# nutdb/nutdb

Hardware: AMD Instinct MI355X
Metric: rows/sec filter->group-by on 1e9-row i64/f64; achieved HBM GB/s vs peak (higher is better)
Workload: dtype i64+f64

## Files before the change

### nutdb_amd/csrc/msd_sort.hip

```cpp
#include <algorithm>
#include <cstdlib>
#include <utility>
#include <vector>

#include "common.hpp"
#include "sort.hpp"

namespace nut {

constexpr int MH_THREADS = 256;
constexpr uint32_t MH_TILE = 1u << 16;
constexpr uint32_t MH_HTILE = 1u << 18;
constexpr int MH_LOADS = 16;
constexpr int MS_THREADS = 1024;
constexpr int MS_ITEMS = 14;
constexpr uint32_t MS_TILE = MS_THREADS * MS_ITEMS;
constexpr int MS_BITS = 9;
constexpr int MS_BINS = 1 << MS_BITS;
static_assert(MS_BINS <= MS_THREADS, "one scan thread per digit");
constexpr int LS_NCLS = 4;
constexpr int LS_S_THREADS = 256, LS_S_ITEMS = 8;
constexpr int LS_M_THREADS = 512, LS_M_ITEMS = 10;
constexpr int LS_M2_THREADS = 512, LS_M2_ITEMS = 12;
constexpr int LS_L_THREADS = 1024, LS_L_ITEMS = 24;
constexpr uint64_t LS_S_CAP = LS_S_THREADS * LS_S_ITEMS;
constexpr uint64_t LS_M_CAP = LS_M_THREADS * LS_M_ITEMS;
constexpr uint64_t LS_M2_CAP = LS_M2_THREADS * LS_M2_ITEMS;
constexpr uint64_t LS_CAP = LS_L_THREADS * LS_L_ITEMS;
__host__ __device__ constexpr int ls_class(uint64_t c) {
  return c <= LS_S_CAP ? 0 : c <= LS_M_CAP ? 1 : c <= LS_M2_CAP ? 2 : c <= LS_CAP ? 3 : LS_NCLS;
}

constexpr uint64_t kSameDst = ~0ull;
struct MsSeg {
  uint64_t start, count;
  uint32_t buf;
  uint32_t aux;
  uint64_t dst = kSameDst;
  uint64_t base = 0;
};
struct MsBufs {
  const uint64_t *in;
  uint64_t *a;
  uint64_t *b;
  uint64_t *c;
};
__device__ __forceinline__ uint64_t ms_dst_off(const MsSeg &g) { return g.dst == kSameDst ? g.start : g.dst; }
struct MsDigit {
  uint64_t base;
  int shift;
  uint32_t mask;
  __device__ __forceinline__ uint32_t operator()(uint64_t k) const { return (uint32_t)((k - base) >> shift) & mask; }
  static constexpr bool kCheck = false;
  static constexpr int kAux = 0;
  __device__ __forceinline__ void setup(uint8_t *) const {}
  __device__ __forceinline__ uint32_t operator()(uint64_t k, const uint8_t *) const { return (*this)(k); }
  uint64_t maxx = ~0ull;
};
struct MsSplit {
  int ns, sbits;
  int64_t e[63];
  const uint8_t *tab;
  static constexpr bool kCheck = false;
  static constexpr int kAux = 4096;
  __device__ __forceinline__ void setup(uint8_t *s) const {
    for (int i = threadIdx.x; i < kAux; i += blockDim.x) s[i] = tab[i];
  }
  __device__ __forceinline__ uint32_t operator()(uint64_t k, const uint8_t *lds) const {
    const uint32_t t = lds[(k ^ 0x8000000000000000ull) >> 52];
    uint32_t d = t & 63u;
    if (t & 0x80u)
      while (d < (uint32_t)ns && (int64_t)k >= e[d]) ++d;
    const uint32_t h = (uint32_t)(k ^ (k >> 29) ^ (k >> 43));
    return (d << sbits) | (h & ((1u << sbits) - 1u));
  }
};
struct MsMap {
  uint64_t base;
  uint32_t mul, lim;
  int t, dshift;
  uint64_t maxx;
  static constexpr bool kCheck = true;
  static constexpr int kAux = 0;
  __device__ __forceinline__ void setup(uint8_t *) const {}
  __device__ __forceinline__ uint32_t operator()(uint64_t k) const {
    return (__umulhi((uint32_t)((k - base) >> t), mul) >> dshift) & (MS_BINS - 1);
  }
  __device__ __forceinline__ uint32_t operator()(uint64_t k, const uint8_t *) const { return (*this)(k); }
};

__device__ __forceinline__ const uint64_t *ms_src(const MsBufs &bf, uint32_t buf) {
  return buf == 0 ? bf.in : (buf == 1 ? bf.a : (buf == 2 ? bf.b : bf.c));
}

template <class DG>
__global__ __launch_bounds__(MH_THREADS) void ms_hist_kernel(MsBufs bf, const MsSeg *__restrict__ segs,
                                                             const uint32_t *__restrict__ tile_seg, DG dg0,
                                                             uint64_t flip, unsigned long long *__restrict__ hist,
                                                             unsigned long long *__restrict__ minmax) {
  __shared__ uint32_t h[MS_BINS];
  __shared__ uint8_t s_aux[DG::kAux > 0 ? DG::kAux : 4];
  const int tid = threadIdx.x;
  dg0.setup(s_aux);
  auto dg = [&](uint64_t k) { return dg0(k, s_aux); };
  for (int i = tid; i < MS_BINS; i += MH_THREADS) h[i] = 0;
  __syncthreads();
  const uint32_t s = tile_seg[blockIdx.x];
  const MsSeg sg = segs[s];
  const uint64_t lo = (uint64_t)(blockIdx.x - sg.aux) * MH_HTILE;
  const uint32_t cnt = (uint32_t)min<uint64_t>(MH_HTILE, sg.count - lo);
  const uint64_t *src = ms_src(bf, sg.buf) + sg.start + lo;
  const uint64_t f = sg.buf == 0 ? flip : 0;
  uint64_t vmin = ~0ull, vmax = 0;
  for (uint32_t i = tid; i < cnt; i += MH_THREADS * MH_LOADS) {
    uint64_t k[MH_LOADS];
#pragma unroll
// ... 5 lines not shown
        atomicAdd(&h[dg(k[j])], 1u);
        vmin = k[j] < vmin ? k[j] : vmin;
        vmax = k[j] > vmax ? k[j] : vmax;
      }
    }
  }
  if (minmax) {
#pragma unroll
    for (int off = 32; off >= 1; off >>= 1) {
      const uint64_t a = __shfl_xor(vmin, off, 64), b = __shfl_xor(vmax, off, 64);
      vmin = a < vmin ? a : vmin;
      vmax = b > vmax ? b : vmax;
    }
    if ((tid & 63) == 0) {
      atomicMin(&minmax[0], (unsigned long long)vmin);
      atomicMax(&minmax[1], (unsigned long long)vmax);
    }
  }
  __syncthreads();
  for (int i = tid; i < MS_BINS; i += MH_THREADS)
    if (h[i]) atomicAdd(&hist[(uint64_t)s * MS_BINS + i], (unsigned long long)h[i]);
}

__device__ __forceinline__ uint64_t *ms_dst(const MsBufs &bf, uint32_t buf, int dst_buf) {
  return dst_buf == 1 ? bf.a : dst_buf == 2 ? bf.b : dst_buf == 3 ? bf.c : (buf == 2 ? bf.a : bf.b);
}
constexpr uint64_t kSkipRun = ~0ull;

template <int H, class DG, int T = MS_THREADS>
__global__ __launch_bounds__(T, 2048 / T) void ms_scatter_kernel(MsBufs bf, const MsSeg *__restrict__ segs,
                                                                   const uint32_t *__restrict__ tile_seg, uint32_t ntiles,
                                                                   DG dg0, uint64_t flip,
                                                                   unsigned long long *__restrict__ cursor,
                                                                   int dst_buf = -1, uint64_t ocap = 0,
                                                                   unsigned long long *__restrict__ oflag = nullptr) {
  constexpr int ITEMS = MS_ITEMS * H;
  constexpr uint32_t STAGE = (uint32_t)T * MS_ITEMS;
  constexpr uint32_t TILE = STAGE * H;
  static_assert(MS_BINS <= T, "one scan thread per digit");
  static_assert(TILE <= 65536, "16-bit ranks");
  __shared__ uint64_t s_keys[STAGE];
  __shared__ uint32_t s_cnt[MS_BINS];
  __shared__ uint32_t s_tex[MS_BINS];
  __shared__ uint64_t s_gb[MS_BINS];
  __shared__ uint32_t s_wsum[MS_BINS / kWave];
  __shared__ uint8_t s_aux[DG::kAux > 0 ? DG::kAux : 4];
  const int tid = threadIdx.x, lane = tid & 63, wave = tid >> 6;
  dg0.setup(s_aux);
  auto dg = [&](uint64_t k) { return dg0(k, s_aux); };
  uint32_t t = blockIdx.x;
  uint64_t key[ITEMS];
  auto load = [&](uint32_t tt, const MsSeg g) {
    const uint64_t lo = (uint64_t)(tt - g.aux) * TILE;
    const uint32_t cn = (uint32_t)min<uint64_t>(TILE, g.count - lo);
    const uint64_t *sp = ms_src(bf, g.buf) + g.start + lo;
    int tq = tid;
    asm volatile("" : "+v"(tq));
#pragma unroll
    for (int i = 0; i < ITEMS; ++i) key[i] = __builtin_nontemporal_load(sp + min((uint32_t)(i * T + tq), cn - 1));
  };
  uint32_t s = tile_seg[t];
  MsSeg sg = segs[s];
  load(t, sg);
  for (;;) {
    int tid_ = tid;
    asm volatile("" : "+v"(tid_));
    const int tid = tid_;
    if (sg.buf == 0 && flip) {
#pragma unroll
      for (int i = 0; i < ITEMS; ++i) key[i] ^= flip;
    }
    const uint64_t lo = (uint64_t)(t - sg.aux) * TILE;
    const uint32_t cnt = (uint32_t)min<uint64_t>(TILE, sg.count - lo);
    uint64_t *dst = ms_dst(bf, sg.buf, dst_buf);
    const uint32_t next = t + gridDim.x;
    const uint32_t ns = next < ntiles ? tile_seg[next] : 0;
    if (tid < MS_BINS) s_cnt[tid] = 0;
    __syncthreads();
    uint32_t rk[ITEMS / 2];
#pragma unroll
    for (int i = 0; i < ITEMS; i += 2) rk[i / 2] = 0;
    bool bad = false;
#pragma unroll
    for (int i = 0; i < ITEMS; ++i) {
      const uint32_t idx = (uint32_t)i * T + tid;
      if (idx < cnt) {
        rk[i / 2] |= atomicAdd(&s_cnt[dg(key[i])], 1u) << (16 * (i & 1));
        if constexpr (DG::kCheck) bad |= key[i] - dg0.base > dg0.maxx;
      }
      if (i % 8 == 7) __builtin_amdgcn_sched_barrier(0);
    }
    if constexpr (DG::kCheck)
      if (__ballot(bad) && lane == 0) atomicOr(oflag, 1ull);
    __syncthreads();
    uint32_t c = 0, incl = 0;
    if (tid < MS_BINS) {
      c = s_cnt[tid];
      incl = c;
#pragma unroll
      for (int off = 1; off < 64; off <<= 1) {
        const uint32_t y = __shfl_up(incl, off, 64);
        if (lane >= off) incl += y;
      }
      if (lane == 63) s_wsum[wave] = incl;
    }
    __syncthreads();
    if (tid < MS_BINS) {
      uint32_t add = 0;
#pragma unroll
      for (int w = 0; w < MS_BINS / kWave; ++w) add += (w < wave) ? s_wsum[w] : 0u;
      const uint32_t tex = incl - c + add;
      s_tex[tid] = tex;
      const uint64_t gb = c ? (uint64_t)atomicAdd(&cursor[(uint64_t)s * MS_BINS + tid], (unsigned long long)c) : 0;
      const bool over = ocap && c && gb + c > ((uint64_t)s * MS_BINS + tid + 1) * ocap;
      if (over) atomicOr(oflag, 1ull);
      s_gb[tid] = over ? kSkipRun : gb - tex;
    }
    __syncthreads();
#pragma unroll
    for (int i = 0; i < ITEMS; i += 2) {
      const uint32_t s0 = s_tex[dg(key[i])] + (rk[i / 2] & 0xFFFFu);
      const uint32_t s1 = s_tex[dg(key[i + 1])] + (rk[i / 2] >> 16);
      rk[i / 2] = (s0 & 0xFFFFu) | (s1 << 16);
      if (i % 8 == 6) __builtin_amdgcn_sched_barrier(0);
    }
    MsSeg nsg = sg;
#pragma unroll
    for (int h = 0; h < H; ++h) {
      if (h) __syncthreads();
#pragma unroll
      for (int i = 0; i < ITEMS; ++i) {
        const uint32_t idx = (uint32_t)i * T + tid;
        const uint32_t slot = (rk[i / 2] >> (16 * (i & 1))) & 0xFFFFu;
        if (idx < cnt && (H == 1 || slot / STAGE == (uint32_t)h)) s_keys[slot % STAGE] = key[i];
      }
      if (h == H - 1 && next < ntiles) {
        __builtin_amdgcn_sched_barrier(0);
        nsg = segs[ns];
        load(next, nsg);
      }
      __syncthreads();
#pragma unroll(H == 1 ? MS_ITEMS : 2)
      for (int i = 0; i < MS_ITEMS; ++i) {
        const uint32_t j = (uint32_t)i * T + tid, jj = j + (uint32_t)h * STAGE;
        if (jj < cnt) {
          const uint64_t k = s_keys[j];
          const uint64_t g = s_gb[dg(k)];
          if (g != kSkipRun) dst[g + jj] = k;
        }
      }
    }
    if (next >= ntiles) break;
    __syncthreads();
    t = next;
    s = ns;
    sg = nsg;
  }
}

__global__ __launch_bounds__(MS_BINS) void ms_plan_kernel(const MsSeg *__restrict__ segs,
                                                          const unsigned long long *__restrict__ hist, int hi,
                                                          uint64_t base,
                                                          unsigned long long *__restrict__ cursor,
                                                          MsSeg *__restrict__ lists, uint64_t cap,
                                                          unsigned int *__restrict__ counts) {
  __shared__ unsigned long long s_wsum[MS_BINS / kWave];
  const int d = threadIdx.x, lane = d & 63, wave = d >> 6;
  const MsSeg sg = segs[blockIdx.x];
  const uint64_t c = hist[(uint64_t)blockIdx.x * MS_BINS + d];
  uint64_t incl = c;
#pragma unroll
  for (int off = 1; off < 64; off <<= 1) {
    const uint64_t y = __shfl_up(incl, off, 64);
    if (lane >= off) incl += y;
  }
  if (lane == 63) s_wsum[wave] = incl;
  __syncthreads();
  uint64_t add = 0;
#pragma unroll
  for (int w = 0; w < MS_BINS / kWave; ++w) add += (w < wave) ? s_wsum[w] : 0ull;
  const uint64_t start = sg.start + incl - c + add;
// ... 777 lines not shown
    launch_class<LS_M_THREADS, LS_M_ITEMS, false>(c, bf, d, n, flip, fb);
  else if (cls == 2)
    launch_class<LS_M2_THREADS, LS_M2_ITEMS, false>(c, bf, d, n, flip, fb);
  else
    launch_class<LS_L_THREADS, LS_L_ITEMS, false>(c, bf, d, n, flip, fb);
  NUT_HIP(hipGetLastError());
  return NUT_OK;
}

static nut_status launch_local(nut_ctx *c, MetaArena &ar, const MsBufs &bf, uint64_t flip,
                               const std::vector<MsSeg> &segs, int cls) {
  if (segs.empty()) return NUT_OK;
  MsSeg *d;
  nut_status s = ar.upload(segs, &d);
  if (s) return s;
  uint32_t *fb = (uint32_t *)ar.alloc((segs.size() + 1) * 4);
  NUT_HIP(hipMemsetAsync(fb, 0, 4, c->stream));
  return launch_local_dev(c, bf, flip, d, (unsigned)segs.size(), fb, cls);
}


static constexpr int ms_halves() { return 2; }

static void launch_scatter(hipStream_t st, unsigned grid, const MsBufs &bf, const MsSeg *segs, const uint32_t *tiles,
                           uint32_t ntiles, const MsDigit &dg, uint64_t flip, unsigned long long *cur) {
  hipLaunchKernelGGL((ms_scatter_kernel<ms_halves(), MsDigit>), dim3(grid), dim3(MS_THREADS), 0, st, bf, segs, tiles, ntiles, dg,
                     flip, cur);
}

static nut_status device_level(nut_ctx *c, MetaArena &ar, const MsBufs &bf, const MsDigit &dg, uint64_t flip,
                               std::vector<MsSeg> &big, std::vector<MsSeg> &over) {
  hipStream_t st = c->stream;
  over.clear();
  std::vector<uint32_t> tiles;
  const uint64_t nht = tile_table(big, MH_HTILE, tiles);
  std::vector<uint32_t> stiles;
  std::vector<MsSeg> sbig = big;
  const uint64_t nst = tile_table(sbig, MS_TILE * ms_halves(), stiles);
  if (nht > 0x7FFFFFFFull || nst > 0x7FFFFFFFull) return fail(NUT_ERR_UNSUPPORTED, "nut_sort_i64: too many tiles");
  const uint64_t ns = big.size(), cap = ns * MS_BINS;
  const size_t hbytes = ns * MS_BINS * 8;
  nut_status s = ar.begin(2 * MetaArena::align(ns * sizeof(MsSeg)) + MetaArena::align(tiles.size() * 4) +
                          MetaArena::align(stiles.size() * 4) + 2 * MetaArena::align(hbytes) +
                          MetaArena::align((LS_NCLS + 1) * cap * sizeof(MsSeg)) +
                          LS_NCLS * MetaArena::align((cap + 1) * 4) + 1024);
  if (s) return s;
  MsSeg *dseg, *dsseg;
  uint32_t *dtile, *dstile;
  if ((s = ar.upload(big, &dseg)) || (s = ar.upload(tiles, &dtile)) || (s = ar.upload(sbig, &dsseg)) ||
      (s = ar.upload(stiles, &dstile)))
    return s;
  unsigned long long *dhist = (unsigned long long *)ar.alloc(hbytes);
  unsigned long long *dcur = (unsigned long long *)ar.alloc(hbytes);
  MsSeg *lists = (MsSeg *)ar.alloc((LS_NCLS + 1) * cap * sizeof(MsSeg));
  unsigned int *counts = (unsigned int *)ar.alloc(4 * (LS_NCLS + 1));
  uint32_t *fb[LS_NCLS];
  for (auto &f : fb) f = (uint32_t *)ar.alloc((cap + 1) * 4);
  NUT_HIP(hipMemsetAsync(dhist, 0, hbytes, st));
  NUT_HIP(hipMemsetAsync(counts, 0, 4 * (LS_NCLS + 1), st));
  uint64_t total = 0;
  for (const MsSeg &sg : big) total += sg.count;
  hipLaunchKernelGGL(ms_hist_kernel<MsDigit>, dim3((unsigned)nht), dim3(MH_THREADS), 0, st, bf, (const MsSeg *)dseg,
                     (const uint32_t *)dtile, dg, flip, dhist, (unsigned long long *)nullptr);
  hipLaunchKernelGGL(ms_plan_kernel, dim3((unsigned)ns), dim3(MS_BINS), 0, st, (const MsSeg *)dseg,
                     (const unsigned long long *)dhist, dg.shift, dg.base, dcur, lists, cap, counts);
  NUT_HIP(hipGetLastError());
  hipEvent_t ev = nullptr;
  NUT_HIP(hipEventCreateWithFlags(&ev, hipEventDisableTiming));
  uint32_t *hc = (uint32_t *)c->host_pinned;
  hipError_t e = hipMemcpyAsync(hc, counts, 4 * (LS_NCLS + 1), hipMemcpyDeviceToHost, st);
  if (e == hipSuccess) e = hipEventRecord(ev, st);
  if (e == hipSuccess)
    launch_scatter(st, (unsigned)std::min<uint64_t>(nst, (uint64_t)c->num_cus), bf, (const MsSeg *)dsseg,
                   (const uint32_t *)dstile, (uint32_t)nst, dg, flip, dcur);
  if (e == hipSuccess) e = hipGetLastError();
  if (e == hipSuccess) e = hipEventSynchronize(ev);
  (void)hipEventDestroy(ev);
  if (e != hipSuccess) return hip_fail(e, "nut_sort_i64 (device-planned level)");
  uint32_t cnt[LS_NCLS + 1];
  for (int k = 0; k <= LS_NCLS; ++k) cnt[k] = hc[k];
  c->sort_bytes += 8 * total + 16 * total;
  ++c->sort_levels;
  for (int cls = LS_NCLS - 1; cls >= 0; --cls)
    if ((s = launch_local_dev(c, bf, flip, lists + (uint64_t)cls * cap, cnt[cls], fb[cls], cls))) return s;
  if (cnt[LS_NCLS]) {
    over.resize(cnt[LS_NCLS]);
    NUT_HIP(hipMemcpyAsync(over.data(), lists + (uint64_t)LS_NCLS * cap, cnt[LS_NCLS] * sizeof(MsSeg),
                           hipMemcpyDeviceToHost, st));
    NUT_HIP(hipStreamSynchronize(st));
  }
  uint64_t over_keys = 0;
  for (const MsSeg &sg : over) over_keys += sg.count;
  c->sort_bytes += 16 * (total - over_keys);
  return NUT_OK;
}

constexpr uint64_t kCappedMin = 1ull << 25;

template <class DG, int T>
static void capped_scatter_t(hipStream_t st, unsigned grid, const MsBufs &bf, const MsSeg *segs, const uint32_t *tiles,
                             uint32_t nt, const DG &dg, uint64_t flip, unsigned long long *cur, int dst_buf,
                             uint64_t ocap, unsigned long long *oflag) {
  hipLaunchKernelGGL((ms_scatter_kernel<ms_halves(), DG, T>), dim3(grid), dim3(T), 0, st, bf, segs, tiles, nt, dg, flip,
                     cur, dst_buf, ocap, oflag);
}
template <class DG>
static void capped_scatter(nut_ctx *c, uint64_t nt, const MsBufs &bf, const MsSeg *segs, const uint32_t *tiles,
                           const DG &dg, uint64_t flip, unsigned long long *cur, int dst_buf, uint64_t ocap,
                           unsigned long long *oflag) {
  const bool half = c->opt[NUT_OPT_SORT_BD] == 512;
  const unsigned grid = (unsigned)std::min<uint64_t>(nt, (uint64_t)c->num_cus * (half ? 2 : 1));
  if (half)
    capped_scatter_t<DG, 512>(c->stream, grid, bf, segs, tiles, (uint32_t)nt, dg, flip, cur, dst_buf, ocap, oflag);
  else
    capped_scatter_t<DG, MS_THREADS>(c->stream, grid, bf, segs, tiles, (uint32_t)nt, dg, flip, cur, dst_buf, ocap, oflag);
}

static bool capped_map(uint64_t lo, uint64_t hi, MsMap &m) {
  if (hi < lo || hi - lo < (1ull << 18)) return false;
  const uint64_t span = hi - lo;
  const int bw = 64 - __builtin_clzll(span);
  const int t = bw > 32 ? bw - 32 : 0;
  const uint64_t lim = span >> t;
  const uint64_t mul = (1ull << 50) / (lim + 1);
  m = MsMap{lo, (uint32_t)mul, (uint32_t)lim, t, 9, ((lim + 1) << t) - 1};
  return true;
}
static uint32_t capped_cell(const MsMap &m, uint64_t k) {
  return (uint32_t)(((uint64_t)(uint32_t)((k - m.base) >> m.t) * m.mul) >> 32);
}

static nut_status msd_sort_capped(nut_ctx *c, const int64_t *in, int64_t *out, uint64_t n, uint64_t flip,
                                  const uint64_t *bounds) {
  hipStream_t st = c->stream;
  constexpr uint32_t kSample = 16384;
  MetaArena ar{c};
  nut_status s = ar.begin(MetaArena::align(kSample * 8) + 1024);
  if (s) return s;
// ... 20 lines not shown
    if (!capped_map(lo, hi, m0)) return NUT_ERR_CAPACITY;
    std::vector<uint32_t> h0(MS_BINS, 0), h1(MS_BINS, 0);
    for (uint64_t k : samp) {
      if (k < lo || k > hi) return NUT_ERR_CAPACITY;
      const uint32_t cell = capped_cell(m0, k);
      ++h0[cell >> MS_BITS];
      ++h1[cell & (MS_BINS - 1)];
    }
    const uint32_t lim = 2 * kSample / MS_BINS;
    for (int d = 0; d < MS_BINS; ++d)
      if (h0[d] > lim || h1[d] > lim) return NUT_ERR_CAPACITY;
  }
  auto reserve = [&](Scratch &sc, size_t bytes) -> nut_status {
    if (sc.reserve(bytes, false) == NUT_OK) return NUT_OK;
    (void)hipGetLastError();
    c->sort_tmp2.release();
    return NUT_ERR_CAPACITY;
  };
  const uint64_t ocap0 = ((n / MS_BINS) * 11 / 10 + 2 * MS_TILE + 31) & ~31ull;
  if ((s = reserve(c->sort_tmp, (size_t)MS_BINS * ocap0 * 8))) return s;
  const MsBufs bf0{(const uint64_t *)in, (uint64_t *)out, (uint64_t *)c->sort_tmp.ptr, nullptr};
  std::vector<MsSeg> one{MsSeg{0, n, 0, 0}};
  std::vector<uint32_t> tiles;
  const uint32_t stile = (c->opt[NUT_OPT_SORT_BD] == 512 ? 512u : (uint32_t)MS_THREADS) * MS_ITEMS * ms_halves();
  const uint64_t nt0 = tile_table(one, stile, tiles);
  if (nt0 > 0x7FFFFFFFull) return fail(NUT_ERR_UNSUPPORTED, "nut_sort_i64: too many tiles");
  std::vector<uint64_t> cur0(MS_BINS + 1, 0);
  for (int d = 0; d < MS_BINS; ++d) cur0[d] = (uint64_t)d * ocap0;
  s = ar.begin(MetaArena::align(sizeof(MsSeg)) + MetaArena::align(tiles.size() * 4) +
               MetaArena::align(cur0.size() * 8));
  if (s) return s;
  MsSeg *dseg;
  uint32_t *dtile;
  uint64_t *dcur0;
  if ((s = ar.upload(one, &dseg)) || (s = ar.upload(tiles, &dtile)) || (s = ar.upload(cur0, &dcur0))) return s;
  const bool ident = m0.base == 0 && m0.t == 32 && m0.mul == (1u << 18);
  unsigned long long *dc0 = (unsigned long long *)dcur0, *of0 = (unsigned long long *)(dcur0 + MS_BINS);
  if (ident)
    capped_scatter(c, nt0, bf0, dseg, dtile, MsDigit{0, 64 - MS_BITS, MS_BINS - 1}, flip, dc0, 2, ocap0, of0);
  else
    capped_scatter(c, nt0, bf0, dseg, dtile, m0, flip, dc0, 2, ocap0, of0);
  NUT_HIP(hipGetLastError());
  std::vector<uint64_t> end0(MS_BINS + 1);
  NUT_HIP(hipMemcpyAsync(end0.data(), dcur0, end0.size() * 8, hipMemcpyDeviceToHost, st));
  NUT_HIP(hipStreamSynchronize(st));
  if (end0[MS_BINS]) return NUT_ERR_CAPACITY;
  std::vector<MsSeg> segs(MS_BINS);
  std::vector<uint64_t> dbase(MS_BINS);
  uint64_t cmax = 0, run = 0;
  for (int d = 0; d < MS_BINS; ++d) {
    const uint64_t cnt = end0[d] - cur0[d];
    segs[d] = MsSeg{cur0[d], cnt, 2, 0};
    dbase[d] = run;
    run += cnt;
    cmax = std::max(cmax, cnt);
  }
  const uint64_t ocap1 = ((cmax / MS_BINS) * 23 / 20 + 64 + 1) & ~1ull;
  if ((s = reserve(c->sort_tmp2, (size_t)MS_BINS * MS_BINS * ocap1 * 8))) return s;
  const MsBufs bf{(const uint64_t *)in, (uint64_t *)out, (uint64_t *)c->sort_tmp.ptr, (uint64_t *)c->sort_tmp2.ptr};
  const uint64_t nt1 = tile_table(segs, stile, tiles);
  if (nt1 > 0x7FFFFFFFull) return fail(NUT_ERR_UNSUPPORTED, "nut_sort_i64: too many tiles");
  const uint64_t nr = (uint64_t)MS_BINS * MS_BINS, lcap = nr;
  std::vector<uint64_t> cur1(nr + 1, 0);
  for (uint64_t r = 0; r < nr; ++r) cur1[r] = r * ocap1;
  s = ar.begin(MetaArena::align(segs.size() * sizeof(MsSeg)) + MetaArena::align(tiles.size() * 4) +
               MetaArena::align(cur1.size() * 8) + MetaArena::align(dbase.size() * 8) +
               MetaArena::align(LS_NCLS * lcap * sizeof(MsSeg)) + LS_NCLS * MetaArena::align((lcap + 1) * 4) + 1024);
  if (s) return s;
  MsSeg *dsegs;
  uint32_t *dt1;
  uint64_t *dcur1, *ddb;
  if ((s = ar.upload(segs, &dsegs)) || (s = ar.upload(tiles, &dt1)) || (s = ar.upload(cur1, &dcur1)) ||
      (s = ar.upload(dbase, &ddb)))
    return s;
  MsSeg *lists = (MsSeg *)ar.alloc(LS_NCLS * lcap * sizeof(MsSeg));
  unsigned int *counts = (unsigned int *)ar.alloc(4 * LS_NCLS);
  uint32_t *fb[LS_NCLS];
  for (auto &f : fb) f = (uint32_t *)ar.alloc((lcap + 1) * 4);
  NUT_HIP(hipMemsetAsync(counts, 0, 4 * LS_NCLS, st));
  MsMap m1 = m0;
  m1.dshift = 0;
  m1.maxx = ~0ull;
  unsigned long long *dc1 = (unsigned long long *)dcur1, *of1 = (unsigned long long *)(dcur1 + nr);
  if (ident)
    capped_scatter(c, nt1, bf, dsegs, dt1, MsDigit{0, 64 - 2 * MS_BITS, MS_BINS - 1}, flip, dc1, 3, ocap1, of1);
  else
    capped_scatter(c, nt1, bf, dsegs, dt1, m1, flip, dc1, 3, ocap1, of1);
  hipLaunchKernelGGL(ms_plan_capped_kernel, dim3(MS_BINS), dim3(MS_BINS), 0, st, (const unsigned long long *)dcur1,
                     (const uint64_t *)ddb, ocap1, m0, lists, lcap, counts, (unsigned long long *)(dcur1 + nr));
  NUT_HIP(hipGetLastError());
  uint64_t *hc = c->host_pinned;
  static_assert(4 * LS_NCLS <= 16, "class counts in the first two pinned words");
  NUT_HIP(hipMemcpyAsync(hc, counts, 4 * LS_NCLS, hipMemcpyDeviceToHost, st));
  NUT_HIP(hipMemcpyAsync(hc + 2, dcur1 + nr, 8, hipMemcpyDeviceToHost, st));
  NUT_HIP(hipStreamSynchronize(st));
  if (hc[2]) return NUT_ERR_CAPACITY;
  const uint32_t *cnt = (const uint32_t *)hc;
  uint32_t ncls[LS_NCLS];
  for (int k = 0; k < LS_NCLS; ++k) ncls[k] = cnt[k];
  for (int cls = LS_NCLS - 1; cls >= 0; --cls)
    if ((s = launch_local_dev(c, bf, flip, lists + (uint64_t)cls * lcap, ncls[cls], fb[cls], cls))) return s;
  c->sort_bytes = 48 * n;
  c->sort_levels = 2;
  return NUT_OK;
}

nut_status msd_sort_i64(nut_ctx *c, const int64_t *in, int64_t *out, uint64_t n, uint64_t flip,
                        const uint64_t *bounds) {
  hipStream_t st = c->stream;
  c->sort_bytes = 0;
// ... 93 lines not shown
    for (size_t i = 0; i < big.size(); ++i) {
      const uint64_t *h = &hist[i * MS_BINS];
      int nz = 0;
      for (int d = 0; d < MS_BINS; ++d) nz += h[d] != 0;
      if (nz <= 1) {
        classify(big[i]);
      } else {
        scat.push_back(big[i]);
        scat_hist.insert(scat_hist.end(), h, h + MS_BINS);
      }
    }
    if (!scat.empty()) {
      cursor.resize(scat.size() * MS_BINS);
      for (size_t i = 0; i < scat.size(); ++i) {
        uint64_t run = scat[i].start;
        const uint32_t nb = scat[i].buf == 2 ? 1u : 2u;
        for (int d = 0; d < MS_BINS; ++d) {
          const uint64_t cnt = scat_hist[i * MS_BINS + d];
          cursor[i * MS_BINS + d] = run;
          if (cnt) classify(MsSeg{run, cnt, nb, 0});
          run += cnt;
        }
      }
      const uint64_t nst = tile_table(scat, MS_TILE * ms_halves(), tiles);
      if (nst > 0x7FFFFFFFull) return fail(NUT_ERR_UNSUPPORTED, "nut_sort_i64: too many tiles");
      s = ar.begin(MetaArena::align(scat.size() * sizeof(MsSeg)) + MetaArena::align(tiles.size() * 4) +
                   MetaArena::align(cursor.size() * 8));
      if (s) return s;
      MsSeg *dsc;
      uint32_t *dt;
      uint64_t *dcur;
      if ((s = ar.upload(scat, &dsc)) || (s = ar.upload(tiles, &dt)) || (s = ar.upload(cursor, &dcur))) return s;
      for (const MsSeg &sg : scat) c->sort_bytes += 16 * sg.count;
      ++c->sort_levels;
      const unsigned sgrid = (unsigned)std::min<uint64_t>(nst, (uint64_t)c->num_cus);
      launch_scatter(st, sgrid, bf, (const MsSeg *)dsc, (const uint32_t *)dt, (uint32_t)nst, dg, flip,
                     (unsigned long long *)dcur);
      NUT_HIP(hipGetLastError());
    }
    big.swap(next);
    const int w = std::min(MS_BITS, hi);
    dg = MsDigit{dg.base, hi - w, (1u << w) - 1u};
    break;
  }
  for (std::vector<MsSeg> over; !big.empty(); big.swap(over)) {
    if (dg.mask == 0) {
      done.insert(done.end(), big.begin(), big.end());
      break;
    }
    if ((s = device_level(c, ar, bf, dg, flip, big, over))) return s;
    const int hi = dg.shift, w = std::min(MS_BITS, hi);
    dg = MsDigit{dg.base, hi - w, (1u << w) - 1u};
  }
  size_t total = 256;
  for (auto &v : small) total += MetaArena::align(v.size() * sizeof(MsSeg)) + MetaArena::align((v.size() + 1) * 4);
  std::vector<uint32_t> ctiles;
  const uint64_t nct = tile_table(done, MH_TILE, ctiles);
  total += MetaArena::align(done.size() * sizeof(MsSeg)) + MetaArena::align(ctiles.size() * 4);
  s = ar.begin(total);
  if (s) return s;
// ... 93 lines not shown
```

Before: 131.9 billion.

## Add carry-granule MSD scatter that writes only aligned runs per digit

Moves the scatter kernel into a header and adds a carry mode. Each block holds back partial runs per digit in LDS and writes to global memory only in multiples of an 8-key granule, flushing the leftovers on a segment's last tile. A blocked tile assignment keeps consecutive tiles of one segment on the same block, so the carries stay valid. The goal is to cut partial-line writes and write amplification in HBM, at the cost of more LDS, a more complex scan, slightly smaller tiles (13 items per thread) and aligned overflow capacity.

```diff
diff --git a/nutdb_amd/csrc/msd_scatter.hpp b/nutdb_amd/csrc/msd_scatter.hpp
--- /dev/null
+++ b/nutdb_amd/csrc/msd_scatter.hpp
@@ -0,0 +1,288 @@
+#pragma once
+#include "common.hpp"
+
+namespace nut {
+
+constexpr int MS_THREADS = 1024;
+constexpr int MS_ITEMS = 14;
+constexpr uint32_t MS_TILE = MS_THREADS * MS_ITEMS;
+constexpr int MS_BITS = 9;
+constexpr int MS_BINS = 1 << MS_BITS;
+static_assert(MS_BINS <= MS_THREADS, "one scan thread per digit");
+
+constexpr uint64_t kSameDst = ~0ull;
+struct MsSeg {
+  uint64_t start, count;
+  uint32_t buf;
+  uint32_t aux;
+  uint64_t dst = kSameDst;
+  uint64_t base = 0;
+};
+struct MsBufs {
+  const uint64_t *in;
+  uint64_t *a;
+  uint64_t *b;
+  uint64_t *c;
+};
+__device__ __forceinline__ uint64_t ms_dst_off(const MsSeg &g) { return g.dst == kSameDst ? g.start : g.dst; }
+struct MsDigit {
+  uint64_t base;
+  int shift;
+  uint32_t mask;
+  __device__ __forceinline__ uint32_t operator()(uint64_t k) const { return (uint32_t)((k - base) >> shift) & mask; }
+  static constexpr bool kCheck = false;
+  static constexpr int kAux = 0;
+  __device__ __forceinline__ void setup(uint8_t *) const {}
+  __device__ __forceinline__ uint32_t operator()(uint64_t k, const uint8_t *) const { return (*this)(k); }
+  uint64_t maxx = ~0ull;
+};
+struct MsSplit {
+  int ns, sbits;
+  int64_t e[63];
+  const uint8_t *tab;
+  static constexpr bool kCheck = false;
+  static constexpr int kAux = 4096;
+  __device__ __forceinline__ void setup(uint8_t *s) const {
+    for (int i = threadIdx.x; i < kAux; i += blockDim.x) s[i] = tab[i];
+  }
+  __device__ __forceinline__ uint32_t operator()(uint64_t k, const uint8_t *lds) const {
+    const uint32_t t = lds[(k ^ 0x8000000000000000ull) >> 52];
+    uint32_t d = t & 63u;
+    if (t & 0x80u)
+      while (d < (uint32_t)ns && (int64_t)k >= e[d]) ++d;
+    const uint32_t h = (uint32_t)(k ^ (k >> 29) ^ (k >> 43));
+    return (d << sbits) | (h & ((1u << sbits) - 1u));
+  }
+};
+struct MsMap {
+  uint64_t base;
+  uint32_t mul, lim;
+  int t, dshift;
+  uint64_t maxx;
+  static constexpr bool kCheck = true;
+  static constexpr int kAux = 0;
+  __device__ __forceinline__ void setup(uint8_t *) const {}
+  __device__ __forceinline__ uint32_t operator()(uint64_t k) const {
+    return (__umulhi((uint32_t)((k - base) >> t), mul) >> dshift) & (MS_BINS - 1);
+  }
+  __device__ __forceinline__ uint32_t operator()(uint64_t k, const uint8_t *) const { return (*this)(k); }
+};
+
+__device__ __forceinline__ const uint64_t *ms_src(const MsBufs &bf, uint32_t buf) {
+  return buf == 0 ? bf.in : (buf == 1 ? bf.a : (buf == 2 ? bf.b : bf.c));
+}
+
+__device__ __forceinline__ uint64_t *ms_dst(const MsBufs &bf, uint32_t buf, int dst_buf) {
+  return dst_buf == 1 ? bf.a : dst_buf == 2 ? bf.b : dst_buf == 3 ? bf.c : (buf == 2 ? bf.a : bf.b);
+}
+constexpr uint64_t kSkipRun = ~0ull;
+
+template <int H, class DG, int T = MS_THREADS, int L = 0, bool BLK = (L > 0), int I1 = MS_ITEMS>
+__global__ __launch_bounds__(T, 2048 / T) void ms_scatter_kernel(MsBufs bf, const MsSeg *__restrict__ segs,
+                                                                   const uint32_t *__restrict__ tile_seg, uint32_t ntiles,
+                                                                   DG dg0, uint64_t flip,
+                                                                   unsigned long long *__restrict__ cursor,
+                                                                   int dst_buf = -1, uint64_t ocap = 0,
+                                                                   unsigned long long *__restrict__ oflag = nullptr) {
+  constexpr int ITEMS = I1 * H;
+  constexpr uint32_t TILE = (uint32_t)T * ITEMS;
+  constexpr uint32_t CARW = L ? L - 1 : 1;
+  constexpr uint32_t STAGE = L ? (TILE + MS_BINS * CARW + H - 1) / H : (uint32_t)T * I1;
+  constexpr int WI = (STAGE + T - 1) / T;
+  static_assert(MS_BINS <= T, "one scan thread per digit");
+  static_assert(L ? STAGE * H + L <= 32768 : TILE <= 65536, "16-bit slots (L > 0: 15 bits)");
+  static_assert(ITEMS % 2 == 0, "ranks in 16-bit pairs");
+  static_assert((L & (L - 1)) == 0 && L <= 128, "the carry granule is a power of two");
+  constexpr uint64_t kM48 = 0xFFFFFFFFFFFFull, kNoRun48 = 0x800000000000ull;
+  __shared__ uint64_t s_keys[STAGE];
+  __shared__ uint32_t s_cnt[MS_BINS];
+  __shared__ uint32_t s_tex[L ? 1 : MS_BINS];
+  __shared__ uint64_t s_gb[MS_BINS];
+  __shared__ uint32_t s_wsum[MS_BINS / kWave];
+  __shared__ uint8_t s_aux[DG::kAux > 0 ? DG::kAux : 4];
+  __shared__ uint64_t s_car[L ? MS_BINS * CARW : 1];
+  __shared__ uint32_t s_ccnt[L ? MS_BINS : 1];
+  __shared__ uint64_t s_sl[L ? MS_BINS : 1];
+  __shared__ uint32_t s_tot[2];
+  const int tid = threadIdx.x, lane0 = tid & 63, wave0 = tid >> 6;
+  dg0.setup(s_aux);
+  auto dg = [&](uint64_t k) { return dg0(k, s_aux); };
+  const uint32_t per = (ntiles + gridDim.x - 1) / gridDim.x;
+  uint32_t t = BLK ? blockIdx.x * per : blockIdx.x;
+  const uint32_t tend = BLK ? min(ntiles, t + per) : ntiles;
+  if (BLK && t >= tend) return;
+  if (L && tid < MS_BINS) s_ccnt[tid] = 0;
+  uint64_t key[ITEMS];
+  auto load = [&](uint32_t tt, const MsSeg g) {
+    const uint64_t lo = (uint64_t)(tt - g.aux) * TILE;
+    const uint32_t cn = (uint32_t)min<uint64_t>(TILE, g.count - lo);
+    const uint64_t *sp = ms_src(bf, g.buf) + g.start + lo;
+    int tq = tid;
+    asm volatile("" : "+v"(tq));
+#pragma unroll
+    for (int i = 0; i < ITEMS; ++i) key[i] = __builtin_nontemporal_load(sp + min((uint32_t)(i * T + tq), cn - 1));
+  };
+  uint32_t s = tile_seg[t];
+  MsSeg sg = segs[s];
+  load(t, sg);
+  for (;;) {
+    int tid_ = tid;
+    asm volatile("" : "+v"(tid_));
+    const int tid = tid_;
+    const int lane = L ? tid & 63 : lane0, wave = L ? tid >> 6 : wave0;
+    if (sg.buf == 0 && flip) {
+#pragma unroll
+      for (int i = 0; i < ITEMS; ++i) key[i] ^= flip;
+    }
+    const uint64_t lo = (uint64_t)(t - sg.aux) * TILE;
+    const uint32_t cnt = (uint32_t)min<uint64_t>(TILE, sg.count - lo);
+    uint64_t *dst = ms_dst(bf, sg.buf, dst_buf);
+    const uint32_t next = BLK ? t + 1 : t + gridDim.x;
+    const uint32_t ns = next < tend ? tile_seg[next] : 0;
+    const bool last = next >= tend || ns != s;
+    if (tid < MS_BINS) s_cnt[tid] = 0;
+    __syncthreads();
+    uint32_t rk[ITEMS / 2];
+#pragma unroll
+    for (int i = 0; i < ITEMS; i += 2) rk[i / 2] = 0;
+    bool bad = false;
+#pragma unroll
+    for (int i = 0; i < ITEMS; ++i) {
+      const uint32_t idx = (uint32_t)i * T + tid;
+      if (idx < cnt) {
+        rk[i / 2] |= atomicAdd(&s_cnt[dg(key[i])], 1u) << (16 * (i & 1));
+        if constexpr (DG::kCheck) bad |= key[i] - dg0.base > dg0.maxx;
+      }
+      if (i % 8 == 7) __builtin_amdgcn_sched_barrier(0);
+    }
+    if constexpr (DG::kCheck)
+      if (__ballot(bad) && lane == 0) atomicOr(oflag, 1ull);
+    __syncthreads();
+    uint32_t c = 0, incl = 0, car = 0, e = 0;
+    if (tid < MS_BINS) {
+      c = s_cnt[tid];
+      if constexpr (L > 0) {
+        car = s_ccnt[tid];
+        e = last ? car + c : (car + c) & ~(uint32_t)(L - 1);
+        c = e | ((car + c - e - (e ? 0 : car)) << 16);
+      }
+      incl = c;
+#pragma unroll
+      for (int off = 1; off < 64; off <<= 1) {
+        const uint32_t y = __shfl_up(incl, off, 64);
+        if (lane >= off) incl += y;
+      }
+      if (lane == 63) s_wsum[wave] = incl;
+    }
+    __syncthreads();
+    if (tid < MS_BINS) {
+      uint32_t add = 0;
+#pragma unroll
+      for (int w = 0; w < MS_BINS / kWave; ++w) add += (w < wave) ? s_wsum[w] : 0u;
+      const uint32_t tex = incl - c + add;
+      if constexpr (L == 0) {
+        s_tex[tid] = tex;
+        const uint64_t gb = c ? (uint64_t)atomicAdd(&cursor[(uint64_t)s * MS_BINS + tid], (unsigned long long)c) : 0;
+        const bool over = ocap && c && gb + c > ((uint64_t)s * MS_BINS + tid + 1) * ocap;
+        if (over) atomicOr(oflag, 1ull);
+        s_gb[tid] = over ? kSkipRun : gb - tex;
+      } else {
+        uint32_t all = 0;
+#pragma unroll
+        for (int w = 0; w < MS_BINS / kWave; ++w) all += s_wsum[w];
+        const uint32_t te = all & 0xFFFFu;
+        const uint32_t lex = tex & 0xFFFFu;
+        const uint32_t stay = e ? 0 : car;
+        const uint32_t tb = te + (tex >> 16) - stay;
+        const uint64_t gb = e ? (uint64_t)atomicAdd(&cursor[(uint64_t)s * MS_BINS + tid], (unsigned long long)e) : 0;
+        const bool over = ocap && e && gb + e > ((uint64_t)s * MS_BINS + tid + 1) * ocap;
+        if (over) atomicOr(oflag, 1ull);
+        s_ccnt[tid] = car + s_cnt[tid] - e;
+        s_gb[tid] = (over ? kNoRun48 : (gb - lex) & kM48) | ((uint64_t)((tb + L) & 0xFFFFu) << 48);
+        s_sl[tid] = (lex + car) | ((lex + e) << 16) | ((uint64_t)((tb - e - lex) & 0xFFFFu) << 32) | ((uint64_t)car << 48) |
+                    ((uint64_t)(e != 0) << 56);
+        if (tid == 0) {
+          s_tot[0] = te;
+          s_tot[1] = te + (all >> 16);
+        }
+      }
+    }
+    __syncthreads();
+    auto slot_of = [&](uint64_t k, uint32_t r) {
+      if constexpr (L == 0) {
+        return s_tex[dg(k)] + r;
+      } else {
+        const uint64_t v = s_sl[dg(k)];
+        const uint32_t s0 = ((uint32_t)v & 0xFFFFu) + r, end = ((uint32_t)v >> 16);
+        return s0 < end ? s0 : s0 + (uint32_t)(v >> 32);
+      }
+    };
+#pragma unroll
+    for (int i = 0; i < ITEMS; i += 2) {
+      const uint32_t s0 = slot_of(key[i], rk[i / 2] & 0xFFFFu);
+      const uint32_t s1 = slot_of(key[i + 1], rk[i / 2] >> 16);
+      rk[i / 2] = (s0 & 0xFFFFu) | (s1 << 16);
+      if (i % (L ? 4 : 8) == (L ? 2 : 6)) __builtin_amdgcn_sched_barrier(0);
+    }
+    MsSeg nsg = sg;
+#pragma unroll
+    for (int h = 0; h < H; ++h) {
+      if (h) __syncthreads();
+#pragma unroll
+      for (int i = 0; i < ITEMS; ++i) {
+        const uint32_t idx = (uint32_t)i * T + tid;
+        const uint32_t slot = (rk[i / 2] >> (16 * (i & 1))) & 0xFFFFu;
+        if (idx < cnt && (H == 1 || slot / STAGE == (uint32_t)h)) s_keys[slot % STAGE] = key[i];
+      }
+      if constexpr (L > 0) {
+        for (uint32_t x = tid; x < MS_BINS * CARW; x += T) {
+          const uint32_t d = x / CARW, p = x - d * CARW;
+          const uint64_t v = s_sl[d];
+          const uint32_t ocar = (uint32_t)(v >> 48) & 0xFFu;
+          const uint32_t slot = ((uint32_t)v & 0xFFFFu) - ocar + p;
+          if ((v >> 56) && p < ocar && slot / STAGE == (uint32_t)h) s_keys[slot % STAGE] = s_car[x];
+        }
+      }
+      if (h == H - 1 && next < tend) {
+        __builtin_amdgcn_sched_barrier(0);
+        nsg = segs[ns];
+        load(next, nsg);
+      }
+      __syncthreads();
+      uint32_t te = 0, ta = 0;
+      if constexpr (L > 0) {
+        te = __builtin_amdgcn_readfirstlane(s_tot[0]);
+        ta = __builtin_amdgcn_readfirstlane(s_tot[1]);
+      }
+#pragma unroll(H == 1 ? WI : 2)
+      for (int i = 0; i < WI; ++i) {
+        const uint32_t j = (uint32_t)i * T + tid, jj = j + (uint32_t)h * STAGE;
+        if constexpr (L == 0) {
+          if (jj < cnt) {
+            const uint64_t k = s_keys[j];
+            const uint64_t g = s_gb[dg(k)];
+            if (g != kSkipRun) dst[g + jj] = k;
+          }
+        } else {
+          if (j < STAGE && jj < ta) {
+            const uint64_t k = s_keys[j];
+            const uint32_t d = dg(k);
+            const uint64_t g = s_gb[d];
+            if (jj < te) {
+              if ((g & kM48) != kNoRun48) dst[(uint64_t)((int64_t)(g << 16) >> 16) + jj] = k;
+            } else {
+              s_car[d * CARW + ((jj + L - (uint32_t)(g >> 48)) & 0xFFFFu)] = k;
+            }
+          }
+        }
+      }
+    }
+    if (next >= tend) break;
+    __syncthreads();
+    t = next;
+    s = ns;
+    sg = nsg;
+  }
+}
+
+}
diff --git a/nutdb_amd/csrc/msd_sort.hip b/nutdb_amd/csrc/msd_sort.hip
--- a/nutdb_amd/csrc/msd_sort.hip
+++ b/nutdb_amd/csrc/msd_sort.hip
@@ -4,6 +4,7 @@
 #include <vector>
 
 #include "common.hpp"
+#include "msd_scatter.hpp"
 #include "sort.hpp"
 
 namespace nut {
@@ -12,12 +13,6 @@
 constexpr uint32_t MH_TILE = 1u << 16;
 constexpr uint32_t MH_HTILE = 1u << 18;
 constexpr int MH_LOADS = 16;
-constexpr int MS_THREADS = 1024;
-constexpr int MS_ITEMS = 14;
-constexpr uint32_t MS_TILE = MS_THREADS * MS_ITEMS;
-constexpr int MS_BITS = 9;
-constexpr int MS_BINS = 1 << MS_BITS;
-static_assert(MS_BINS <= MS_THREADS, "one scan thread per digit");
 constexpr int LS_NCLS = 4;
 constexpr int LS_S_THREADS = 256, LS_S_ITEMS = 8;
 constexpr int LS_M_THREADS = 512, LS_M_ITEMS = 10;
@@ -31,67 +26,6 @@
   return c <= LS_S_CAP ? 0 : c <= LS_M_CAP ? 1 : c <= LS_M2_CAP ? 2 : c <= LS_CAP ? 3 : LS_NCLS;
 }
 
-constexpr uint64_t kSameDst = ~0ull;
-struct MsSeg {
-  uint64_t start, count;
-  uint32_t buf;
-  uint32_t aux;
-  uint64_t dst = kSameDst;
-  uint64_t base = 0;
-};
-struct MsBufs {
-  const uint64_t *in;
-  uint64_t *a;
-  uint64_t *b;
-  uint64_t *c;
-};
-__device__ __forceinline__ uint64_t ms_dst_off(const MsSeg &g) { return g.dst == kSameDst ? g.start : g.dst; }
-struct MsDigit {
-  uint64_t base;
-  int shift;
-  uint32_t mask;
-  __device__ __forceinline__ uint32_t operator()(uint64_t k) const { return (uint32_t)((k - base) >> shift) & mask; }
-  static constexpr bool kCheck = false;
-  static constexpr int kAux = 0;
-  __device__ __forceinline__ void setup(uint8_t *) const {}
-  __device__ __forceinline__ uint32_t operator()(uint64_t k, const uint8_t *) const { return (*this)(k); }
-  uint64_t maxx = ~0ull;
-};
-struct MsSplit {
-  int ns, sbits;
-  int64_t e[63];
-  const uint8_t *tab;
-  static constexpr bool kCheck = false;
-  static constexpr int kAux = 4096;
-  __device__ __forceinline__ void setup(uint8_t *s) const {
-    for (int i = threadIdx.x; i < kAux; i += blockDim.x) s[i] = tab[i];
-  }
-  __device__ __forceinline__ uint32_t operator()(uint64_t k, const uint8_t *lds) const {
-    const uint32_t t = lds[(k ^ 0x8000000000000000ull) >> 52];
-    uint32_t d = t & 63u;
-    if (t & 0x80u)
-      while (d < (uint32_t)ns && (int64_t)k >= e[d]) ++d;
-    const uint32_t h = (uint32_t)(k ^ (k >> 29) ^ (k >> 43));
-    return (d << sbits) | (h & ((1u << sbits) - 1u));
-  }
-};
-struct MsMap {
-  uint64_t base;
-  uint32_t mul, lim;
-  int t, dshift;
-  uint64_t maxx;
-  static constexpr bool kCheck = true;
-  static constexpr int kAux = 0;
-  __device__ __forceinline__ void setup(uint8_t *) const {}
-  __device__ __forceinline__ uint32_t operator()(uint64_t k) const {
-    return (__umulhi((uint32_t)((k - base) >> t), mul) >> dshift) & (MS_BINS - 1);
-  }
-  __device__ __forceinline__ uint32_t operator()(uint64_t k, const uint8_t *) const { return (*this)(k); }
-};
-
-__device__ __forceinline__ const uint64_t *ms_src(const MsBufs &bf, uint32_t buf) {
-  return buf == 0 ? bf.in : (buf == 1 ? bf.a : (buf == 2 ? bf.b : bf.c));
-}
 
 template <class DG>
 __global__ __launch_bounds__(MH_THREADS) void ms_hist_kernel(MsBufs bf, const MsSeg *__restrict__ segs,
@@ -143,141 +77,6 @@
     if (h[i]) atomicAdd(&hist[(uint64_t)s * MS_BINS + i], (unsigned long long)h[i]);
 }
 
-__device__ __forceinline__ uint64_t *ms_dst(const MsBufs &bf, uint32_t buf, int dst_buf) {
-  return dst_buf == 1 ? bf.a : dst_buf == 2 ? bf.b : dst_buf == 3 ? bf.c : (buf == 2 ? bf.a : bf.b);
-}
-constexpr uint64_t kSkipRun = ~0ull;
-
-template <int H, class DG, int T = MS_THREADS>
-__global__ __launch_bounds__(T, 2048 / T) void ms_scatter_kernel(MsBufs bf, const MsSeg *__restrict__ segs,
-                                                                   const uint32_t *__restrict__ tile_seg, uint32_t ntiles,
-                                                                   DG dg0, uint64_t flip,
-                                                                   unsigned long long *__restrict__ cursor,
-                                                                   int dst_buf = -1, uint64_t ocap = 0,
-                                                                   unsigned long long *__restrict__ oflag = nullptr) {
-  constexpr int ITEMS = MS_ITEMS * H;
-  constexpr uint32_t STAGE = (uint32_t)T * MS_ITEMS;
-  constexpr uint32_t TILE = STAGE * H;
-  static_assert(MS_BINS <= T, "one scan thread per digit");
-  static_assert(TILE <= 65536, "16-bit ranks");
-  __shared__ uint64_t s_keys[STAGE];
-  __shared__ uint32_t s_cnt[MS_BINS];
-  __shared__ uint32_t s_tex[MS_BINS];
-  __shared__ uint64_t s_gb[MS_BINS];
-  __shared__ uint32_t s_wsum[MS_BINS / kWave];
-  __shared__ uint8_t s_aux[DG::kAux > 0 ? DG::kAux : 4];
-  const int tid = threadIdx.x, lane = tid & 63, wave = tid >> 6;
-  dg0.setup(s_aux);
-  auto dg = [&](uint64_t k) { return dg0(k, s_aux); };
-  uint32_t t = blockIdx.x;
-  uint64_t key[ITEMS];
-  auto load = [&](uint32_t tt, const MsSeg g) {
-    const uint64_t lo = (uint64_t)(tt - g.aux) * TILE;
-    const uint32_t cn = (uint32_t)min<uint64_t>(TILE, g.count - lo);
-    const uint64_t *sp = ms_src(bf, g.buf) + g.start + lo;
-    int tq = tid;
-    asm volatile("" : "+v"(tq));
-#pragma unroll
-    for (int i = 0; i < ITEMS; ++i) key[i] = __builtin_nontemporal_load(sp + min((uint32_t)(i * T + tq), cn - 1));
-  };
-  uint32_t s = tile_seg[t];
-  MsSeg sg = segs[s];
-  load(t, sg);
-  for (;;) {
-    int tid_ = tid;
-    asm volatile("" : "+v"(tid_));
-    const int tid = tid_;
-    if (sg.buf == 0 && flip) {
-#pragma unroll
-      for (int i = 0; i < ITEMS; ++i) key[i] ^= flip;
-    }
-    const uint64_t lo = (uint64_t)(t - sg.aux) * TILE;
-    const uint32_t cnt = (uint32_t)min<uint64_t>(TILE, sg.count - lo);
-    uint64_t *dst = ms_dst(bf, sg.buf, dst_buf);
-    const uint32_t next = t + gridDim.x;
-    const uint32_t ns = next < ntiles ? tile_seg[next] : 0;
-    if (tid < MS_BINS) s_cnt[tid] = 0;
-    __syncthreads();
-    uint32_t rk[ITEMS / 2];
-#pragma unroll
-    for (int i = 0; i < ITEMS; i += 2) rk[i / 2] = 0;
-    bool bad = false;
-#pragma unroll
-    for (int i = 0; i < ITEMS; ++i) {
-      const uint32_t idx = (uint32_t)i * T + tid;
-      if (idx < cnt) {
-        rk[i / 2] |= atomicAdd(&s_cnt[dg(key[i])], 1u) << (16 * (i & 1));
-        if constexpr (DG::kCheck) bad |= key[i] - dg0.base > dg0.maxx;
-      }
-      if (i % 8 == 7) __builtin_amdgcn_sched_barrier(0);
-    }
-    if constexpr (DG::kCheck)
-      if (__ballot(bad) && lane == 0) atomicOr(oflag, 1ull);
-    __syncthreads();
-    uint32_t c = 0, incl = 0;
-    if (tid < MS_BINS) {
-      c = s_cnt[tid];
-      incl = c;
-#pragma unroll
-      for (int off = 1; off < 64; off <<= 1) {
-        const uint32_t y = __shfl_up(incl, off, 64);
-        if (lane >= off) incl += y;
-      }
-      if (lane == 63) s_wsum[wave] = incl;
-    }
-    __syncthreads();
-    if (tid < MS_BINS) {
-      uint32_t add = 0;
-#pragma unroll
-      for (int w = 0; w < MS_BINS / kWave; ++w) add += (w < wave) ? s_wsum[w] : 0u;
-      const uint32_t tex = incl - c + add;
-      s_tex[tid] = tex;
-      const uint64_t gb = c ? (uint64_t)atomicAdd(&cursor[(uint64_t)s * MS_BINS + tid], (unsigned long long)c) : 0;
-      const bool over = ocap && c && gb + c > ((uint64_t)s * MS_BINS + tid + 1) * ocap;
-      if (over) atomicOr(oflag, 1ull);
-      s_gb[tid] = over ? kSkipRun : gb - tex;
-    }
-    __syncthreads();
-#pragma unroll
-    for (int i = 0; i < ITEMS; i += 2) {
-      const uint32_t s0 = s_tex[dg(key[i])] + (rk[i / 2] & 0xFFFFu);
-      const uint32_t s1 = s_tex[dg(key[i + 1])] + (rk[i / 2] >> 16);
-      rk[i / 2] = (s0 & 0xFFFFu) | (s1 << 16);
-      if (i % 8 == 6) __builtin_amdgcn_sched_barrier(0);
-    }
-    MsSeg nsg = sg;
-#pragma unroll
-    for (int h = 0; h < H; ++h) {
-      if (h) __syncthreads();
-#pragma unroll
-      for (int i = 0; i < ITEMS; ++i) {
-        const uint32_t idx = (uint32_t)i * T + tid;
-        const uint32_t slot = (rk[i / 2] >> (16 * (i & 1))) & 0xFFFFu;
-        if (idx < cnt && (H == 1 || slot / STAGE == (uint32_t)h)) s_keys[slot % STAGE] = key[i];
-      }
-      if (h == H - 1 && next < ntiles) {
-        __builtin_amdgcn_sched_barrier(0);
-        nsg = segs[ns];
-        load(next, nsg);
-      }
-      __syncthreads();
-#pragma unroll(H == 1 ? MS_ITEMS : 2)
-      for (int i = 0; i < MS_ITEMS; ++i) {
-        const uint32_t j = (uint32_t)i * T + tid, jj = j + (uint32_t)h * STAGE;
-        if (jj < cnt) {
-          const uint64_t k = s_keys[j];
-          const uint64_t g = s_gb[dg(k)];
-          if (g != kSkipRun) dst[g + jj] = k;
-        }
-      }
-    }
-    if (next >= ntiles) break;
-    __syncthreads();
-    t = next;
-    s = ns;
-    sg = nsg;
-  }
-}
 
 __global__ __launch_bounds__(MS_BINS) void ms_plan_kernel(const MsSeg *__restrict__ segs,
                                                           const unsigned long long *__restrict__ hist, int hi,
@@ -1101,10 +900,21 @@
 
 static constexpr int ms_halves() { return 2; }
 
-static void launch_scatter(hipStream_t st, unsigned grid, const MsBufs &bf, const MsSeg *segs, const uint32_t *tiles,
-                           uint32_t ntiles, const MsDigit &dg, uint64_t flip, unsigned long long *cur) {
-  hipLaunchKernelGGL((ms_scatter_kernel<ms_halves(), MsDigit>), dim3(grid), dim3(MS_THREADS), 0, st, bf, segs, tiles, ntiles, dg,
-                     flip, cur);
+constexpr int MS_CARRY = 8;
+constexpr int MS_CITEMS = 13;
+constexpr uint32_t MS_CTILE = (uint32_t)MS_THREADS * MS_CITEMS * ms_halves();
+
+template <class DG>
+static void launch_carry_scatter(hipStream_t st, unsigned grid, bool blocked, const MsBufs &bf, const MsSeg *segs,
+                                 const uint32_t *tiles, uint32_t ntiles, const DG &dg, uint64_t flip,
+                                 unsigned long long *cur, int dst_buf = -1, uint64_t ocap = 0,
+                                 unsigned long long *oflag = nullptr) {
+  if (blocked)
+    hipLaunchKernelGGL((ms_scatter_kernel<ms_halves(), DG, MS_THREADS, MS_CARRY, true, MS_CITEMS>), dim3(grid),
+                       dim3(MS_THREADS), 0, st, bf, segs, tiles, ntiles, dg, flip, cur, dst_buf, ocap, oflag);
+  else
+    hipLaunchKernelGGL((ms_scatter_kernel<ms_halves(), DG, MS_THREADS, MS_CARRY, false, MS_CITEMS>), dim3(grid),
+                       dim3(MS_THREADS), 0, st, bf, segs, tiles, ntiles, dg, flip, cur, dst_buf, ocap, oflag);
 }
 
 static nut_status device_level(nut_ctx *c, MetaArena &ar, const MsBufs &bf, const MsDigit &dg, uint64_t flip,
@@ -1115,7 +925,7 @@
   const uint64_t nht = tile_table(big, MH_HTILE, tiles);
   std::vector<uint32_t> stiles;
   std::vector<MsSeg> sbig = big;
-  const uint64_t nst = tile_table(sbig, MS_TILE * ms_halves(), stiles);
+  const uint64_t nst = tile_table(sbig, MS_CTILE, stiles);
   if (nht > 0x7FFFFFFFull || nst > 0x7FFFFFFFull) return fail(NUT_ERR_UNSUPPORTED, "nut_sort_i64: too many tiles");
   const uint64_t ns = big.size(), cap = ns * MS_BINS;
   const size_t hbytes = ns * MS_BINS * 8;
@@ -1150,8 +960,8 @@
   hipError_t e = hipMemcpyAsync(hc, counts, 4 * (LS_NCLS + 1), hipMemcpyDeviceToHost, st);
   if (e == hipSuccess) e = hipEventRecord(ev, st);
   if (e == hipSuccess)
-    launch_scatter(st, (unsigned)std::min<uint64_t>(nst, (uint64_t)c->num_cus), bf, (const MsSeg *)dsseg,
-                   (const uint32_t *)dstile, (uint32_t)nst, dg, flip, dcur);
+    launch_carry_scatter(st, (unsigned)std::min<uint64_t>(nst, (uint64_t)c->num_cus), ns > 1, bf, (const MsSeg *)dsseg,
+                         (const uint32_t *)dstile, (uint32_t)nst, dg, flip, dcur);
   if (e == hipSuccess) e = hipGetLastError();
   if (e == hipSuccess) e = hipEventSynchronize(ev);
   (void)hipEventDestroy(ev);
@@ -1184,15 +994,15 @@
                      cur, dst_buf, ocap, oflag);
 }
 template <class DG>
-static void capped_scatter(nut_ctx *c, uint64_t nt, const MsBufs &bf, const MsSeg *segs, const uint32_t *tiles,
-                           const DG &dg, uint64_t flip, unsigned long long *cur, int dst_buf, uint64_t ocap,
-                           unsigned long long *oflag) {
+static void capped_scatter(nut_ctx *c, uint64_t nt, bool blocked, const MsBufs &bf, const MsSeg *segs,
+                           const uint32_t *tiles, const DG &dg, uint64_t flip, unsigned long long *cur, int dst_buf,
+                           uint64_t ocap, unsigned long long *oflag) {
   const bool half = c->opt[NUT_OPT_SORT_BD] == 512;
   const unsigned grid = (unsigned)std::min<uint64_t>(nt, (uint64_t)c->num_cus * (half ? 2 : 1));
   if (half)
     capped_scatter_t<DG, 512>(c->stream, grid, bf, segs, tiles, (uint32_t)nt, dg, flip, cur, dst_buf, ocap, oflag);
   else
-    capped_scatter_t<DG, MS_THREADS>(c->stream, grid, bf, segs, tiles, (uint32_t)nt, dg, flip, cur, dst_buf, ocap, oflag);
+    launch_carry_scatter(c->stream, grid, blocked, bf, segs, tiles, (uint32_t)nt, dg, flip, cur, dst_buf, ocap, oflag);
 }
 
 static bool capped_map(uint64_t lo, uint64_t hi, MsMap &m) {
@@ -1259,7 +1069,7 @@
   const MsBufs bf0{(const uint64_t *)in, (uint64_t *)out, (uint64_t *)c->sort_tmp.ptr, nullptr};
   std::vector<MsSeg> one{MsSeg{0, n, 0, 0}};
   std::vector<uint32_t> tiles;
-  const uint32_t stile = (c->opt[NUT_OPT_SORT_BD] == 512 ? 512u : (uint32_t)MS_THREADS) * MS_ITEMS * ms_halves();
+  const uint32_t stile = c->opt[NUT_OPT_SORT_BD] == 512 ? 512u * MS_ITEMS * ms_halves() : MS_CTILE;
   const uint64_t nt0 = tile_table(one, stile, tiles);
   if (nt0 > 0x7FFFFFFFull) return fail(NUT_ERR_UNSUPPORTED, "nut_sort_i64: too many tiles");
   std::vector<uint64_t> cur0(MS_BINS + 1, 0);
@@ -1274,9 +1084,9 @@
   const bool ident = m0.base == 0 && m0.t == 32 && m0.mul == (1u << 18);
   unsigned long long *dc0 = (unsigned long long *)dcur0, *of0 = (unsigned long long *)(dcur0 + MS_BINS);
   if (ident)
-    capped_scatter(c, nt0, bf0, dseg, dtile, MsDigit{0, 64 - MS_BITS, MS_BINS - 1}, flip, dc0, 2, ocap0, of0);
+    capped_scatter(c, nt0, false, bf0, dseg, dtile, MsDigit{0, 64 - MS_BITS, MS_BINS - 1}, flip, dc0, 2, ocap0, of0);
   else
-    capped_scatter(c, nt0, bf0, dseg, dtile, m0, flip, dc0, 2, ocap0, of0);
+    capped_scatter(c, nt0, false, bf0, dseg, dtile, m0, flip, dc0, 2, ocap0, of0);
   NUT_HIP(hipGetLastError());
   std::vector<uint64_t> end0(MS_BINS + 1);
   NUT_HIP(hipMemcpyAsync(end0.data(), dcur0, end0.size() * 8, hipMemcpyDeviceToHost, st));
@@ -1292,7 +1102,7 @@
     run += cnt;
     cmax = std::max(cmax, cnt);
   }
-  const uint64_t ocap1 = ((cmax / MS_BINS) * 23 / 20 + 64 + 1) & ~1ull;
+  const uint64_t ocap1 = ((cmax / MS_BINS) * 23 / 20 + 64 + MS_CARRY - 1) & ~(uint64_t)(MS_CARRY - 1);
   if ((s = reserve(c->sort_tmp2, (size_t)MS_BINS * MS_BINS * ocap1 * 8))) return s;
   const MsBufs bf{(const uint64_t *)in, (uint64_t *)out, (uint64_t *)c->sort_tmp.ptr, (uint64_t *)c->sort_tmp2.ptr};
   const uint64_t nt1 = tile_table(segs, stile, tiles);
@@ -1320,9 +1130,9 @@
   m1.maxx = ~0ull;
   unsigned long long *dc1 = (unsigned long long *)dcur1, *of1 = (unsigned long long *)(dcur1 + nr);
   if (ident)
-    capped_scatter(c, nt1, bf, dsegs, dt1, MsDigit{0, 64 - 2 * MS_BITS, MS_BINS - 1}, flip, dc1, 3, ocap1, of1);
+    capped_scatter(c, nt1, true, bf, dsegs, dt1, MsDigit{0, 64 - 2 * MS_BITS, MS_BINS - 1}, flip, dc1, 3, ocap1, of1);
   else
-    capped_scatter(c, nt1, bf, dsegs, dt1, m1, flip, dc1, 3, ocap1, of1);
+    capped_scatter(c, nt1, true, bf, dsegs, dt1, m1, flip, dc1, 3, ocap1, of1);
   hipLaunchKernelGGL(ms_plan_capped_kernel, dim3(MS_BINS), dim3(MS_BINS), 0, st, (const unsigned long long *)dcur1,
                      (const uint64_t *)ddb, ocap1, m0, lists, lcap, counts, (unsigned long long *)(dcur1 + nr));
   NUT_HIP(hipGetLastError());
@@ -1462,7 +1272,7 @@
           run += cnt;
         }
       }
-      const uint64_t nst = tile_table(scat, MS_TILE * ms_halves(), tiles);
+      const uint64_t nst = tile_table(scat, MS_CTILE, tiles);
       if (nst > 0x7FFFFFFFull) return fail(NUT_ERR_UNSUPPORTED, "nut_sort_i64: too many tiles");
       s = ar.begin(MetaArena::align(scat.size() * sizeof(MsSeg)) + MetaArena::align(tiles.size() * 4) +
                    MetaArena::align(cursor.size() * 8));
@@ -1474,8 +1284,8 @@
       for (const MsSeg &sg : scat) c->sort_bytes += 16 * sg.count;
       ++c->sort_levels;
       const unsigned sgrid = (unsigned)std::min<uint64_t>(nst, (uint64_t)c->num_cus);
-      launch_scatter(st, sgrid, bf, (const MsSeg *)dsc, (const uint32_t *)dt, (uint32_t)nst, dg, flip,
-                     (unsigned long long *)dcur);
+      launch_carry_scatter(st, sgrid, scat.size() > 1, bf, (const MsSeg *)dsc, (const uint32_t *)dt, (uint32_t)nst, dg,
+                           flip, (unsigned long long *)dcur);
       NUT_HIP(hipGetLastError());
     }
     big.swap(next);
```

After: 131.8 billion. About the same (-0.1%).
